# PereUbu7/Variational-Self-Organizing-Maps

Hardware: NVIDIA B200
Metric: train_samples_per_s (higher is better)
Workload: dtype f32

## Files before the change

### include/vsom_b200.h

```cpp
#ifndef VSOM_B200_H
#define VSOM_B200_H

#include <stddef.h>
#include <stdint.h>

#ifdef __cplusplus
extern "C" {
#endif

#if defined(__GNUC__)
#define VSOM_API __attribute__((visibility("default")))
#else
#define VSOM_API
#endif

typedef struct vsom_ctx vsom_ctx;

typedef enum vsom_status
{
    VSOM_OK = 0,
    VSOM_ERR_INVALID = -1,
    VSOM_ERR_CUDA = -2,
    VSOM_ERR_UNSUPPORTED = -3,
    VSOM_ERR_TIMEOUT = -4,
// ... 29 lines not shown
VSOM_API int vsom_peer_export_planes(vsom_ctx *ctx, unsigned char handle[64]);
VSOM_API int vsom_peer_import_planes(vsom_ctx *ctx, int rank, const unsigned char handle[64]);
VSOM_API int vsom_peer_attach(vsom_ctx *ctx, int rank, vsom_ctx *peer);
VSOM_API int vsom_shard_rows(const vsom_ctx *ctx, int *block_rows, int *local_rows, int *global_rows);
VSOM_API const char *vsom_last_error(const vsom_ctx *ctx);
VSOM_API int vsom_model_length(int d_in, int transform);
VSOM_API int vsom_depth(const vsom_ctx *ctx);
VSOM_API int vsom_node_count(const vsom_ctx *ctx);
VSOM_API void *vsom_stream(const vsom_ctx *ctx);
VSOM_API int vsom_synchronize(vsom_ctx *ctx);
VSOM_API uint64_t vsom_launch_count(const vsom_ctx *ctx);
VSOM_API int vsom_planes_resident(const vsom_ctx *ctx);

VSOM_API int vsom_debug_profile(vsom_ctx *ctx, int enable);
VSOM_API int vsom_debug_last_train_fast(const vsom_ctx *ctx);
VSOM_API int vsom_debug_phase_cycles(vsom_ctx *ctx, double out[5]);
VSOM_API int vsom_debug_phase_cycles_raw(vsom_ctx *ctx, double out[8]);
VSOM_API int vsom_debug_die_aware(const vsom_ctx *ctx);

VSOM_API int vsom_debug_measure_peaks(vsom_ctx *ctx, double out[4]);

VSOM_API int vsom_upload_state(vsom_ctx *ctx, const float *mean, const float *S, const float *sigma, const float *weight, const uint64_t *hits);
VSOM_API int vsom_download_state(vsom_ctx *ctx, float *mean, float *S, float *sigma, float *weight, uint64_t *hits);

#define VSOM_LINEAR_INIT_SLAB_ROWS 16384
VSOM_API int vsom_linear_init(vsom_ctx *ctx, const float *x, size_t n, double *out_mean, double *out_lambda, double *out_axes);
VSOM_API int vsom_debug_linear_init_phases(const vsom_ctx *ctx, double out[4]);

#define VSOM_CLUSTER_BLOCK 1024
typedef enum vsom_cluster_weighting
// ... 52 lines not shown
```

### variational-self-organizing-maps_b200/binding.py

```python
from __future__ import annotations

import ctypes as C
import os
import re

import numpy as np

from . import build as _build

STANDARD, MEDIAN, CLR = 0, 1, 2
EXPONENTIAL, INVERSE_PROPORTIONAL = 0, 1
ORDER_REFERENCE, ORDER_LANES, ORDER_EIGEN_SSE = 0, 1, 2
CLUSTER_UNIFORM, CLUSTER_HITS = 0, 1

_f32p = C.POINTER(C.c_float)
_f64p = C.POINTER(C.c_double)
_u32p = C.POINTER(C.c_uint32)
_u64p = C.POINTER(C.c_uint64)
_i32p = C.POINTER(C.c_int32)
_vp = C.c_void_p

_PROTOS = {
    "vsom_create": (C.c_int, [C.POINTER(_vp), C.c_int, C.c_int, C.c_int, C.c_int, C.c_int, C.c_int]),
    "vsom_destroy": (None, [_vp]),
# ... 2 lines not shown
    "vsom_peer_import": (C.c_int, [_vp, C.c_int, C.c_char_p]),
    "vsom_peer_export_planes": (C.c_int, [_vp, C.c_char_p]),
    "vsom_peer_import_planes": (C.c_int, [_vp, C.c_int, C.c_char_p]),
    "vsom_peer_attach": (C.c_int, [_vp, C.c_int, _vp]),
    "vsom_shard_rows": (C.c_int, [_vp, C.POINTER(C.c_int), C.POINTER(C.c_int), C.POINTER(C.c_int)]),
    "vsom_last_error": (C.c_char_p, [_vp]),
    "vsom_model_length": (C.c_int, [C.c_int, C.c_int]),
    "vsom_depth": (C.c_int, [_vp]),
    "vsom_node_count": (C.c_int, [_vp]),
    "vsom_stream": (_vp, [_vp]),
    "vsom_synchronize": (C.c_int, [_vp]),
    "vsom_launch_count": (C.c_uint64, [_vp]),
    "vsom_planes_resident": (C.c_int, [_vp]),
    "vsom_debug_profile": (C.c_int, [_vp, C.c_int]),
    "vsom_debug_last_train_fast": (C.c_int, [_vp]),
    "vsom_debug_phase_cycles_raw": (C.c_int, [_vp, _f64p]),
    "vsom_debug_die_aware": (C.c_int, [_vp]),
    "vsom_debug_measure_peaks": (C.c_int, [_vp, _f64p]),
    "vsom_debug_phase_cycles": (C.c_int, [_vp, _f64p]),
    "vsom_upload_state": (C.c_int, [_vp, _f32p, _f32p, _f32p, _f32p, _u64p]),
    "vsom_download_state": (C.c_int, [_vp, _f32p, _f32p, _f32p, _f32p, _u64p]),
    "vsom_get_node": (C.c_int, [_vp, C.c_size_t, _f32p, _f32p]),
    "vsom_linear_init": (C.c_int, [_vp, _f32p, C.c_size_t, _f64p, _f64p, _f64p]),
    "vsom_debug_linear_init_phases": (C.c_int, [_vp, _f64p]),
    "vsom_debug_cluster_phases": (C.c_int, [_vp, _f64p]),
    "vsom_cluster_nodes": (C.c_int, [_vp, C.c_int, C.c_uint64, C.c_int, C.c_int, _i32p, _f64p, _f64p, _f64p, C.POINTER(C.c_int), C.POINTER(C.c_int)]),
    "vsom_train_chunk": (C.c_int, [_vp, _f32p, C.c_size_t, C.c_double, C.c_double, C.c_int, _u64p, _u32p, _f32p, _f32p]),
    "vsom_train_chunk_device": (C.c_int, [_vp, _vp, C.c_size_t, C.c_double, C.c_double, C.c_int, _vp, _vp]),
    "vsom_batch_epoch": (C.c_int, [_vp, _f32p, C.c_size_t, C.c_double, C.c_int, _u64p, _f32p]),
    "vsom_find_bmu": (C.c_int, [_vp, _f32p, C.c_size_t, C.c_uint64, _u32p, _f32p]),
# ... 350 lines not shown
        return dict(zip(names, out.tolist()))

    def measure_peaks(self):
        out = np.zeros(4, np.float64)
        self._check(lib().vsom_debug_measure_peaks(self._h, _p(out, _f64p)))
        return {"smem_gbs": out[0], "smem_gbs_per_sm": out[1], "l2_gbs": out[2], "l2_set_mib": out[3]}

    @property
    def die_aware(self) -> bool:
        return bool(lib().vsom_debug_die_aware(self._h))

    @property
    def last_train_fast(self) -> bool:
        return bool(lib().vsom_debug_last_train_fast(self._h))

    def synchronize(self):
        self._check(lib().vsom_synchronize(self._h))

    @property
    def stream(self) -> int:
        return int(lib().vsom_stream(self._h) or 0)

    @property
    def launch_count(self) -> int:
        return int(lib().vsom_launch_count(self._h))

    @property
    def planes_resident(self) -> bool:
        return bool(lib().vsom_planes_resident(self._h))
```

### variational-self-organizing-maps_b200/csrc/capi.cu

```cuda
#include "common.cuh"

#include <cstdlib>

#include <algorithm>
#include <cstdio>
#include <cstring>

namespace vsom
{

static std::string g_createError;

int set_error(vsom_ctx *ctx, int code, const std::string &msg)
{
    if (ctx)
        ctx->err = msg;
    else
        g_createError = msg;
    return code;
}

int cuda_fail(vsom_ctx *ctx, cudaError_t e, const char *what, const char *file, int line)
{
    char buf[512];
// ... 320 lines not shown
        }
    }
    if (ctx->stream)
        cudaStreamDestroy(ctx->stream);
    delete ctx;
}

const char *vsom_last_error(const vsom_ctx *ctx) { return ctx ? ctx->err.c_str() : g_createError.c_str(); }
int vsom_depth(const vsom_ctx *ctx) { return ctx ? ctx->Dm : 0; }
int vsom_node_count(const vsom_ctx *ctx) { return ctx ? ctx->N : 0; }
void *vsom_stream(const vsom_ctx *ctx) { return ctx ? static_cast<void *>(ctx->stream) : nullptr; }
uint64_t vsom_launch_count(const vsom_ctx *ctx) { return ctx ? ctx->launches : 0; }
int vsom_planes_resident(const vsom_ctx *ctx) { return ctx ? ctx->k1.resident : 0; }

int vsom_debug_last_train_fast(const vsom_ctx *ctx) { return ctx && ctx->lastPlan == &ctx->k1f ? 1 : 0; }

int vsom_debug_profile(vsom_ctx *ctx, int enable)
{
    if (!ctx)
        return VSOM_ERR_INVALID;
    VSOM_CUDA(ctx, cudaSetDevice(ctx->device));
    VSOM_CUDA(ctx, cudaStreamSynchronize(ctx->stream));
    if (enable && !ctx->profDev)
    {
        VSOM_CUDA(ctx, cudaMalloc(&ctx->profDev, sizeof(long long) * 8 * ctx->numSMs));
        VSOM_CUDA(ctx, cudaMemset(ctx->profDev, 0, sizeof(long long) * 8 * ctx->numSMs));
    }
    else if (!enable && ctx->profDev)
    {
        VSOM_CUDA(ctx, cudaFree(ctx->profDev));
// ... 618 lines not shown
```

### variational-self-organizing-maps_b200/csrc/common.cuh

```cuda
#pragma once

#include <cuda.h>
#include <cuda_runtime.h>
#include <stdint.h>

#include <cmath>
#include <string>
#include <vector>

#include "vsom_b200.h"

namespace vsom
{

typedef unsigned long long u64;

constexpr size_t kMaxGridY = 65535;

struct LutEntry
{
    double nw;
    float cexp;
    float nwf;
};
// ... 55 lines not shown
    const void *scanMap;
};

struct StepPlan
{
    void (*kernel[2])(const StepParams) = {};
    int grid = 0;
    int threads = 0;
    size_t smem = 0;
    size_t smemCap = 0;
    int resident = 0;
    int smStride = 0;
    int lanesPerNode = 0;
    int profStride = 0;
    unsigned char profFold[5] = {};
};

}

struct vsom_ctx
{
    int device = 0;
    int W = 0, H = 0, N = 0, Din = 0, Dm = 0, Dr = 0, P = 0;
    int rank = 0, world = 1;
    int localN = 0;
    int shardBlock = 0, localRows = 0;
    std::vector<int> localRowY;
    float *peerMean[8] = {};
    bool peerMeanOpened[8] = {};
    vsom::u64 *rankSlots = nullptr;
// ... 19 lines not shown
    int *errFlag = nullptr;
    vsom::LutEntry *lut = nullptr;
    size_t lutCap = 0;
    std::vector<vsom::LutEntry> lutHost;
    double lutEta = -1, lutSigma = -1;
    int lutW = 0, lutH = 0;
    void *stage[10] = {};
    size_t stageCap[10] = {};
    bool trainEnqueued = false;
    bool poisoned = false;
    unsigned long long tcStats[3] = {0, 0, 0};
    int lastScoreTier = 0;
    uint64_t launches = 0;
    vsom::StepPlan k1, k1f;
    const vsom::StepPlan *lastPlan = nullptr;
    unsigned *winTab = nullptr;
    double winSigma = -1;
    vsom::u64 *rowPool = nullptr;
    int *rowMeta = nullptr;
    int dieAware = 0;
    vsom::u64 *distTag = nullptr;
    int scanBufs = 0, scanSeg = 0, scanNSeg = 0;
    void *scanMapDev = nullptr;
    void *umTab = nullptr;
    int umTiles = 0;
    long long *profDev = nullptr;
    size_t profSamples = 0;
    double linInitPhase[4] = {};
    double clusterPhase[5] = {};
    std::string err;
// ... 565 lines not shown
```

### variational-self-organizing-maps_b200/csrc/online_step.cu

```cuda
#include "common.cuh"

#include <cmath>
#include <cstdlib>
#include <string>

namespace vsom
{

constexpr int kThreads = 1024;
constexpr int kWarps = kThreads / 32;
constexpr int kMaxSlotsPerLane = 5;
constexpr size_t kStaticSmem = 1024;

template <int TR>
__device__ __forceinline__ void update_element(float xv, float c, float nwf, float &m, float &S)
{
    auto stepper = [](float d) { return TR == VSOM_MEDIAN ? median_sign(d) : d; };
    const float d0 = stepper(__fsub_rn(xv, m));
    const float m1 = __fadd_rn(m, __fmul_rn(c, d0));
    const float d1 = stepper(__fsub_rn(xv, m1));
    S = __fadd_rn(S, __fmul_rn(nwf, __fmul_rn(d0, d1)));
    m = m1;
}

// ... 974 lines not shown
        return set_error(ctx, VSOM_ERR_INVALID, "online step: decay must be Exponential or InverseProportional");
    if (n == 0)
        return VSOM_OK;
    if (ctx->world > 1)
        for (int r = 0; r < ctx->world; ++r)
            if (!ctx->peerSlots[r])
                return set_error(ctx, VSOM_ERR_INVALID, "online step: sharded context without vsom_peer_import for every rank");
    if (ctx->poisoned)
        return set_error(ctx, VSOM_ERR_TIMEOUT, "online step: an earlier chunk of this context aborted (a CTA or a rank never published its key); "
                                                "the map and the cross-rank step counter are no longer consistent — re-create the context");
    int rc = build_lut(ctx, eta, sigma);
    if (rc)
        return rc;
    const bool fast = ctx->k1f.grid && n < (1ull << 32) - 1;
    const StepPlan &plan = fast ? ctx->k1f : ctx->k1;
    VSOM_CUDA(ctx, cudaMemsetAsync(ctx->errFlag, 0, sizeof(int), ctx->stream));

    StepParams p{};
    p.W = ctx->W;
    p.H = ctx->H;
    p.shardBlock = ctx->shardBlock;
    p.nodeCount = ctx->localN;
    p.order = ctx->order;
    p.world = ctx->world;
    p.rank = ctx->rank;
    p.rankSlots = ctx->rankSlots;
    for (int r = 0; r < 8; ++r)
        p.peerSlots[r] = ctx->peerSlots[r];
    p.stepBase = ctx->stepBase;
    p.Din = ctx->Din;
// ... 20 lines not shown
    p.timeoutCycles = 4000000000ll;
    {
        const char *e = getenv("VSOM_PEER_TIMEOUT_S");
        const double secs = e && atof(e) > 0 ? atof(e) : 60.0;
        p.peerTimeoutCycles = static_cast<long long>(secs * 2.0e9);
    }
    p.localSearch = localSearch ? 1 : 0;
    p.lastIn = lastInDev;
    p.prof = ctx->profDev;
    p.xVec = (ctx->Din % 4 == 0 && (reinterpret_cast<uintptr_t>(xDev) & 15) == 0) ? 1 : 0;
    p.resident = plan.resident;
    p.smStride = plan.smStride;
    p.lanesPerNode = plan.lanesPerNode;
    p.lutCount = ctx->lutW * ctx->lutH;
    const size_t lutBytes = sizeof(LutEntry) * static_cast<size_t>(p.lutCount);
    p.lutSmem = plan.smem + lutBytes <= plan.smemCap ? 1 : 0;
    rc = fast ? prepare_online_step_fast(ctx, p, sigma) : prepare_online_step(ctx, p);
    if (rc)
        return rc;

    void *args[] = {&p};
    VSOM_CUDA(ctx, cudaLaunchCooperativeKernel(reinterpret_cast<void *>(plan.kernel[p.prof ? 1 : 0]), dim3(plan.grid), dim3(plan.threads), args,
                                               plan.smem + (p.lutSmem ? lutBytes : 0), ctx->stream));
    ctx->lastPlan = &plan;
    ctx->profSamples = n;
    ctx->launches += 1;
    ctx->stepBase += n;
    return VSOM_OK;
}

}
```

### variational-self-organizing-maps_b200/csrc/online_step_fast.cu

```cuda
#include "common.cuh"

#include <algorithm>
#include <cmath>
#include <cstdio>
#include <cstdlib>
#include <mutex>

namespace vsom
{

constexpr int kFThreads = 512;
constexpr int kFWarps = kFThreads / 32;
constexpr int kFMaxSlotsPerLane = 5;
constexpr int kFMaxCtas = 32 * kFMaxSlotsPerLane;
constexpr size_t kFStaticSmem = 4096;
constexpr int kFPoolBlocks = 1024;
constexpr int kWalkReplicas = 1;

__device__ __forceinline__ void named_bar_sync(int id, int threads) { asm volatile("bar.sync %0, %1;" ::"r"(id), "r"(threads) : "memory"); }
__device__ __forceinline__ void cp_async_commit() { asm volatile("cp.async.commit_group;" ::: "memory"); }

__device__ __forceinline__ u64 pk(float2 v) { return (static_cast<u64>(__float_as_uint(v.y)) << 32) | __float_as_uint(v.x); }
__device__ __forceinline__ float2 unpk(u64 v) { return make_float2(__uint_as_float(static_cast<unsigned>(v)), __uint_as_float(static_cast<unsigned>(v >> 32))); }
__device__ __forceinline__ float2 sub2(float2 a, float2 b)
// ... 126 lines not shown
    float rest[8] = {0.f, 0.f, 0.f, 0.f, 0.f, 0.f, 0.f, 0.f};
    if (nrest)
    {
        const float4 u = r4[2 * n8], v = r4[2 * n8 + 1];
        rest[0] = u.x;
        rest[1] = u.y;
        rest[2] = u.z;
        rest[3] = u.w;
        rest[4] = v.x;
        rest[5] = v.y;
        rest[6] = v.z;
        rest[7] = v.w;
    }
    return acc.finish(rest, nrest);
}
__device__ __forceinline__ float chain_lanes8(const float *row, int Dr, int c)
{
    const int n8 = Dr >> 3;
    float a = 0.0f;
    const float *q = row + c;
    int b = 0;
    if (n8 >= 8)
    {
        float v[8], w[8];
#pragma unroll
        for (int j = 0; j < 8; ++j)
            v[j] = q[8 * j];
#pragma unroll 1
        for (b = 8; b + 8 <= n8; b += 8)
        {
// ... 2 lines not shown
                w[j] = q[8 * (b + j)];
#pragma unroll
            for (int j = 0; j < 8; ++j)
                a = __fadd_rn(a, v[j]);
#pragma unroll
            for (int j = 0; j < 8; ++j)
                v[j] = w[j];
        }
#pragma unroll
        for (int j = 0; j < 8; ++j)
            a = __fadd_rn(a, v[j]);
    }
#pragma unroll 1
    for (; b < n8; ++b)
        a = __fadd_rn(a, q[8 * b]);
    float r = __fadd_rn(a, __shfl_xor_sync(0xffffffffu, a, 4));
    const int nrest = Dr & 7;
    const float *rest = row + (n8 << 3);
    int k = 0;
    if (nrest >= 4)
    {
        r = __fadd_rn(r, rest[c & 3]);
        k = 4;
    }
    r = __fadd_rn(r, __shfl_xor_sync(0xffffffffu, r, 2));
    r = __fadd_rn(r, __shfl_xor_sync(0xffffffffu, r, 1));
    for (; k < nrest; ++k)
        r = __fadd_rn(r, rest[k]);
    return r;
}
__device__ __forceinline__ float chain_any(const float *row, int n16, int Dr, int eigen) { return eigen ? chain_terms_eigen(row, Dr) : chain_terms(row, n16); }

__device__ __forceinline__ float4 clr_terms4(const float4 a, const float4 b, const float4 xi, const float4 xj)
{
    float4 t;
    float r = clr_residual(a.x, b.x, xi.x, xj.x);
    t.x = __fmul_rn(r, r);
    r = clr_residual(a.y, b.y, xi.y, xj.y);
    t.y = __fmul_rn(r, r);
    r = clr_residual(a.z, b.z, xi.z, xj.z);
    t.z = __fmul_rn(r, r);
    r = clr_residual(a.w, b.w, xi.w, xj.w);
    t.w = __fmul_rn(r, r);
    return t;
}

__device__ __forceinline__ u64 make_key_xy(float d, unsigned x, unsigned y, unsigned tag)
{
    unsigned bits = __float_as_uint(d);
    if (d != d)
        bits = (x | y) == 0 ? 0u : 0x7fffffffu;
    return (static_cast<u64>(bits) << 32) | (static_cast<u64>(y) << 20) | (static_cast<u64>(x) << 8) | tag;
}

__device__ __forceinline__ unsigned ld_relaxed_gpu_u32(const unsigned *p)
{
    unsigned v;
    asm volatile("ld.relaxed.gpu.global.u32 %0, [%1];" : "=r"(v) : "l"(p) : "memory");
    return v;
}

template <int TR, int IPW, bool PROF>
__global__ void __launch_bounds__(kFThreads, 1) online_step_fast_kernel(const StepParams p)
{
    constexpr int NI = IPW > 0 ? IPW : 1;
    extern __shared__ __align__(16) unsigned char smemRaw[];
    __shared__ u64 *sRowPtr[2][kFMaxCtas];
    __shared__ u64 sWarpKey[kFWarps];
    __shared__ int sPend[2];
    __shared__ unsigned sBmu;
    __shared__ int sAbort;
    __shared__ long long sProf[8];

    const int G = gridDim.x, b = blockIdx.x, tid = threadIdx.x, lane = tid & 31, warp = tid >> 5;
// ... 28 lines not shown
    ushort4 *pairS = reinterpret_cast<ushort4 *>(sBase + (IPW > 0 ? 0 : static_cast<size_t>(Lmax) * rstride));
    float *gS = reinterpret_cast<float *>(pairS + (kClr ? 2 * (Ppad >> 2) : 0));
    LutEntry *lutS = reinterpret_cast<LutEntry *>(gS + (kClr ? 6 * Ppad : 0));
    if (kClr)
    {
        unsigned short *pt = reinterpret_cast<unsigned short *>(pairS);
        const unsigned short zeroAt = static_cast<unsigned short>(XS - 4);
        for (int q = tid; q < Ppad; q += kFThreads)
        {
            pt[q] = q < p.P ? p.pairI[q] : zeroAt;
            pt[Ppad + q] = q < p.P ? p.pairJ[q] : zeroAt;
        }
    }

    if (tid == 0)
    {
        unsigned smid;
        asm volatile("mov.u32 %0, %%smid;" : "=r"(smid));
        const int die = p.dieOfSm[smid & 255];
        const unsigned idx = atomicAdd(p.rowCtr + die, 1u);
        p.rowOf[b] = die * kFMaxCtas + static_cast<int>(idx);
        __threadfence();
        atomicAdd(p.rowCtr + 2, 1u);
        const long long b0 = clock64();
        while (ld_relaxed_gpu_u32(p.rowCtr + 2) < static_cast<unsigned>(G))
            if (clock64() - b0 > p.timeoutCycles)
            {
                *p.err = 1;
                break;
            }
        __threadfence();
    }
    if (p.lutSmem)
        for (int i = tid; i < p.lutCount; i += kFThreads)
            lutS[i] = p.lut[i];
    for (int i = tid; i < p.W; i += kFThreads)
        winX[i] = p.winTab[i];
    for (int i = tid; i < p.H; i += kFThreads)
        winY[i] = p.winTab[p.W + i];
    for (int l = tid; l < Lpad; l += kFThreads)
    {
        hitsS[l] = 0;
        touchedS[l] = 0;
    }
    for (int k = tid; k < 4 * XS; k += kFThreads)
        xs[k] = 0.0f;
    for (int k = tid; k < stride; k += kFThreads)
// ... 60 lines not shown
    const int myL = LPN == 8 ? tid >> 3 : tid, mySub = LPN == 8 ? tid & 7 : 0;
    const bool inScan = myL < L;
    const bool hasNode = inScan && mySub == 0;
    unsigned myX = 0, myY = 0;
    float myW = 0.0f;
    unsigned myTouched = 0;
    if (hasNode)
    {
        const unsigned node = static_cast<unsigned>(p.node0 + myL * G + b);
        myX = node % static_cast<unsigned>(p.W);
        myY = node / static_cast<unsigned>(p.W);
        myW = p.weight[static_cast<size_t>(myL) * G + b];
    }
    const float *myTerms = tBase + (inScan ? myL : 0) * stride;
    __syncthreads();
    for (int i = tid; i < 2 * G; i += kFThreads)
    {
        const int d = i >> 1, buf = i & 1;
        const int r = p.rowOf[d];
        sRowPtr[buf][d] = p.rowPool + static_cast<size_t>(p.rowBlocks[2 * r + buf]) * 256;
    }

    constexpr int kPrefetchWarp = kFWarps - 2;
    const float *xsrc = p.x;
    int xdst = 0;
    auto prefetch = [&]() {
        float *dst = xs + xdst;
        if (p.xVec)
        {
#pragma unroll 1
            for (int k = lane * 4; k < p.Din; k += 128)
                cp_async16(dst + k, xsrc + k);
        }
        else
        {
#pragma unroll 1
// ... 118 lines not shown
            key = warp_min_key(key);
            if (nSW > 1)
            {
                if (lane == 0)
                    sWarpKey[warp] = key;
                named_bar_sync(1, nSW * 32);
            }
            unsigned bxy = 0;
            bool abort = false;
            if (warp == 0)
            {
                if (nSW > 1)
                    key = warp_min_key(lane < nSW ? sWarpKey[lane] : ~0ull);
                if (PROF && tid == 0)
                    c2 = clock64();
                u64 *const *rp = sRowPtr[par];
#pragma unroll
                for (int j = 0; j < kFMaxSlotsPerLane; ++j)
                    if (lane + 32 * j < G)
                        st_relaxed_gpu(rp[lane + 32 * j] + b, key);
                const u64 *row = rp[b];
                const u64 filler = (~0ull << 8) | tag;
                u64 m;
                long long t0 = 0;
                if (p.pollDelay > 0)
                {
                    const long long w0 = clock64();
                    while (clock64() - w0 < p.pollDelay)
                        ;
                }
                for (unsigned round = 0;; ++round)
                {
                    u64 v[kFMaxSlotsPerLane];
#pragma unroll
                    for (int j = 0; j < kFMaxSlotsPerLane; ++j)
                    {
                        const int i = lane + 32 * j;
                        v[j] = i < G ? ld_relaxed_gpu(row + i) : filler;
                    }
                    m = ~0ull;
                    int ok = 1;
#pragma unroll
                    for (int j = 0; j < kFMaxSlotsPerLane; ++j)
                    {
                        ok &= (static_cast<unsigned>(v[j] & 0xff) == tag);
                        m = u64_min(m, v[j]);
                    }
                    if (__all_sync(0xffffffffu, ok))
                        break;
                    if ((round & 63) == 63)
                    {
                        if (t0 == 0)
                            t0 = clock64();
                        else if (__any_sync(0xffffffffu, clock64() - t0 > p.timeoutCycles))
                        {
                            abort = true;
                            break;
                        }
                    }
                }
                m = warp_min_key(m);
                bxy = static_cast<unsigned>(m >> 8) & 0xffffffu;
                if (p.localSearch && !abort)
                {
                    if (lane == 0)
                    {
                        const u64 *dt = p.distTag + (static_cast<size_t>(par) * kWalkReplicas + (b % kWalkReplicas)) * p.nodeCount;
                        const unsigned want = t + 1u;
                        const unsigned bmu = local_bmu_walk(
                            [&](u64 i) {
                                u64 w = ld_relaxed_gpu(dt + i);
                                if (static_cast<unsigned>(w) != want)
                                {
                                    const long long w0 = clock64();
                                    do
                                        w = ld_relaxed_gpu(dt + i);
// ... 235 lines not shown
            for (int k = lane; k < p.Dm; k += 32)
            {
                const int ks = kClr ? (k < p.P ? k : Ppad + (k - p.P)) : k;
                const float sv = sBase[l * rstride + ks];
                p.mean[g + k] = mBase[l * rstride + ks];
                p.S[g + k] = sv;
                if (vis)
                    p.sigma[g + k] = lazy_sigma(sv, w);
            }
        }
    if (PROF && p.prof && tid == 0)
        for (int i = 0; i < 8; ++i)
            p.prof[static_cast<size_t>(b) * 8 + i] = sProf[i];
}

__global__ void die_pingpong_kernel(u64 *f1, u64 *f2, int ctaA, int ctaB, int iters, u64 base, long long *out, int *smids)
{
    if (threadIdx.x != 0)
        return;
    const int b = blockIdx.x;
    if (b != ctaA && b != ctaB)
        return;
    unsigned smid;
    asm volatile("mov.u32 %0, %%smid;" : "=r"(smid));
    smids[b == ctaA ? 0 : 1] = static_cast<int>(smid);
    const long long t0 = clock64();
    const long long limit = 400000000ll;
    for (int t = 1; t <= iters; ++t)
    {
        const u64 v = base + t;
// ... 93 lines not shown
    return bytes;
}

typedef void (*FastKernel)(const StepParams);
static FastKernel pick_fast(int transform, int ipw, bool prof)
{
    if (transform == VSOM_CLR)
        return prof ? online_step_fast_kernel<VSOM_CLR, 0, true> : online_step_fast_kernel<VSOM_CLR, 0, false>;
#define VSOM_FK(TR, I) {online_step_fast_kernel<TR, I, false>, online_step_fast_kernel<TR, I, true>}
#define VSOM_FKS(TR) {VSOM_FK(TR, 0), VSOM_FK(TR, 1), VSOM_FK(TR, 2), VSOM_FK(TR, 4)}
    static const FastKernel table[2][4][2] = {VSOM_FKS(VSOM_STANDARD), VSOM_FKS(VSOM_MEDIAN)};
#undef VSOM_FKS
#undef VSOM_FK
    const int slot = ipw == 4 ? 3 : ipw;
    return table[transform == VSOM_MEDIAN ? 1 : 0][slot][prof ? 1 : 0];
}

struct DieMap
{
    bool tried = false, valid = false;
    int dieOfSm[256] = {};
    int count[2] = {0, 0};
};
static DieMap g_dieMap[64];
static std::mutex g_dieMapMutex;

static bool split_bimodal(std::vector<float> v, float &thr)
{
    if (v.size() < 8)
        return false;
// ... 233 lines not shown
    {
        FastKernel k = pick_fast(ctx->transform, ipw, prof != 0);
        if (cudaFuncSetAttribute(k, cudaFuncAttributeMaxDynamicSharedMemorySize, ctx->smemOptin - static_cast<int>(kFStaticSmem)) != cudaSuccess)
        {
            cudaGetLastError();
            return;
        }
        int perSm = 0;
        if (cudaOccupancyMaxActiveBlocksPerMultiprocessor(&perSm, k, kFThreads, bytes) != cudaSuccess || perSm < 1)
        {
            cudaGetLastError();
            return;
        }
        pl.kernel[prof] = k;
    }
    pl.grid = G;
    pl.threads = kFThreads;
    pl.smem = bytes;
    pl.smemCap = static_cast<size_t>(ctx->smemOptin) - kFStaticSmem;
    pl.resident = 1;
    pl.smStride = stride;
    pl.lanesPerNode = ctx->order == VSOM_ORDER_EIGEN_SSE && Lmax * 8 <= kFThreads && (Lmax * 8 <= 32 || ctx->Dr >= 256) ? 8 : 1;
    pl.profStride = 8;
    const unsigned char fold[5] = {0, 0x03, 0x04, 0x18, 0x60};
    std::copy(fold, fold + 5, pl.profFold);
    ctx->k1f = pl;
}

static int build_window_table(vsom_ctx *ctx, double sigma)
{
// ... 50 lines not shown
```

Baseline: 473,100.

## Add warp-specialized pipelined online step kernel with register-resident nodes

Adds a new cooperative online-training kernel that keeps each node's mean and S in registers, with two nodes per node warp. A dedicated exchange warp performs the cross-CTA BMU min-exchange while node warps prefetch samples through a cp.async ring and compute the next sample's distances, synchronising over named barriers. This is meant to overlap distance computation, sample loading and the global exchange latency, and to avoid shared-memory round trips for node state. It is only used for standard/median transforms with Eigen-SSE ordering, Dr a multiple of 8 up to 256, and small per-CTA node counts. It adds a large, complex code path with a separate reduction order that must match the existing one.

```diff
diff --git a/include/vsom_b200.h b/include/vsom_b200.h
--- a/include/vsom_b200.h
+++ b/include/vsom_b200.h
@@ -67,6 +67,7 @@
 
 VSOM_API int vsom_debug_profile(vsom_ctx *ctx, int enable);
 VSOM_API int vsom_debug_last_train_fast(const vsom_ctx *ctx);
+VSOM_API int vsom_debug_last_online_body(const vsom_ctx *ctx);
 VSOM_API int vsom_debug_phase_cycles(vsom_ctx *ctx, double out[5]);
 VSOM_API int vsom_debug_phase_cycles_raw(vsom_ctx *ctx, double out[8]);
 VSOM_API int vsom_debug_die_aware(const vsom_ctx *ctx);
diff --git a/variational-self-organizing-maps_b200/binding.py b/variational-self-organizing-maps_b200/binding.py
--- a/variational-self-organizing-maps_b200/binding.py
+++ b/variational-self-organizing-maps_b200/binding.py
@@ -40,6 +40,7 @@
     "vsom_planes_resident": (C.c_int, [_vp]),
     "vsom_debug_profile": (C.c_int, [_vp, C.c_int]),
     "vsom_debug_last_train_fast": (C.c_int, [_vp]),
+    "vsom_debug_last_online_body": (C.c_int, [_vp]),
     "vsom_debug_phase_cycles_raw": (C.c_int, [_vp, _f64p]),
     "vsom_debug_die_aware": (C.c_int, [_vp]),
     "vsom_debug_measure_peaks": (C.c_int, [_vp, _f64p]),
@@ -420,6 +421,10 @@
     def last_train_fast(self) -> bool:
         return bool(lib().vsom_debug_last_train_fast(self._h))
 
+    @property
+    def last_online_body(self):
+        return {0: "generic", 1: "fast", 2: "pipelined"}.get(int(lib().vsom_debug_last_online_body(self._h)))
+
     def synchronize(self):
         self._check(lib().vsom_synchronize(self._h))
 
diff --git a/variational-self-organizing-maps_b200/csrc/capi.cu b/variational-self-organizing-maps_b200/csrc/capi.cu
--- a/variational-self-organizing-maps_b200/csrc/capi.cu
+++ b/variational-self-organizing-maps_b200/csrc/capi.cu
@@ -358,6 +358,12 @@
 int vsom_planes_resident(const vsom_ctx *ctx) { return ctx ? ctx->k1.resident : 0; }
 
 int vsom_debug_last_train_fast(const vsom_ctx *ctx) { return ctx && ctx->lastPlan == &ctx->k1f ? 1 : 0; }
+int vsom_debug_last_online_body(const vsom_ctx *ctx)
+{
+    if (!ctx || !ctx->lastPlan)
+        return -1;
+    return ctx->lastPlan != &ctx->k1f ? 0 : ctx->lastPipelined ? 2 : 1;
+}
 
 int vsom_debug_profile(vsom_ctx *ctx, int enable)
 {
diff --git a/variational-self-organizing-maps_b200/csrc/common.cuh b/variational-self-organizing-maps_b200/csrc/common.cuh
--- a/variational-self-organizing-maps_b200/csrc/common.cuh
+++ b/variational-self-organizing-maps_b200/csrc/common.cuh
@@ -93,6 +93,8 @@
     int lanesPerNode = 0;
     int profStride = 0;
     unsigned char profFold[5] = {};
+    void (*pipelined[2])(const StepParams) = {};
+    size_t pipelinedSmem = 0;
 };
 
 }
@@ -142,6 +144,7 @@
     uint64_t launches = 0;
     vsom::StepPlan k1, k1f;
     const vsom::StepPlan *lastPlan = nullptr;
+    int lastPipelined = 0;
     unsigned *winTab = nullptr;
     double winSigma = -1;
     vsom::u64 *rowPool = nullptr;
diff --git a/variational-self-organizing-maps_b200/csrc/online_step.cu b/variational-self-organizing-maps_b200/csrc/online_step.cu
--- a/variational-self-organizing-maps_b200/csrc/online_step.cu
+++ b/variational-self-organizing-maps_b200/csrc/online_step.cu
@@ -1012,6 +1012,8 @@
         return rc;
     const bool fast = ctx->k1f.grid && n < (1ull << 32) - 1;
     const StepPlan &plan = fast ? ctx->k1f : ctx->k1;
+    const bool pipelined = fast && !localSearch && plan.pipelined[0];
+    const size_t smem = pipelined ? plan.pipelinedSmem : plan.smem;
     VSOM_CUDA(ctx, cudaMemsetAsync(ctx->errFlag, 0, sizeof(int), ctx->stream));
 
     StepParams p{};
@@ -1062,15 +1064,16 @@
     p.lanesPerNode = plan.lanesPerNode;
     p.lutCount = ctx->lutW * ctx->lutH;
     const size_t lutBytes = sizeof(LutEntry) * static_cast<size_t>(p.lutCount);
-    p.lutSmem = plan.smem + lutBytes <= plan.smemCap ? 1 : 0;
+    p.lutSmem = smem + lutBytes <= plan.smemCap ? 1 : 0;
     rc = fast ? prepare_online_step_fast(ctx, p, sigma) : prepare_online_step(ctx, p);
     if (rc)
         return rc;
 
     void *args[] = {&p};
-    VSOM_CUDA(ctx, cudaLaunchCooperativeKernel(reinterpret_cast<void *>(plan.kernel[p.prof ? 1 : 0]), dim3(plan.grid), dim3(plan.threads), args,
-                                               plan.smem + (p.lutSmem ? lutBytes : 0), ctx->stream));
+    VSOM_CUDA(ctx, cudaLaunchCooperativeKernel(reinterpret_cast<void *>((pipelined ? plan.pipelined : plan.kernel)[p.prof ? 1 : 0]), dim3(plan.grid),
+                                               dim3(plan.threads), args, smem + (p.lutSmem ? lutBytes : 0), ctx->stream));
     ctx->lastPlan = &plan;
+    ctx->lastPipelined = pipelined ? 1 : 0;
     ctx->profSamples = n;
     ctx->launches += 1;
     ctx->stepBase += n;
diff --git a/variational-self-organizing-maps_b200/csrc/online_step_fast.cu b/variational-self-organizing-maps_b200/csrc/online_step_fast.cu
--- a/variational-self-organizing-maps_b200/csrc/online_step_fast.cu
+++ b/variational-self-organizing-maps_b200/csrc/online_step_fast.cu
@@ -164,6 +164,22 @@
     }
     return acc.finish(rest, nrest);
 }
+__device__ __forceinline__ float eigen_lanes8_finish(float a, const float *rest, int nrest, int c)
+{
+    float r = __fadd_rn(a, __shfl_xor_sync(0xffffffffu, a, 4));
+    int k = 0;
+    if (nrest >= 4)
+    {
+        r = __fadd_rn(r, rest[c & 3]);
+        k = 4;
+    }
+    r = __fadd_rn(r, __shfl_xor_sync(0xffffffffu, r, 2));
+    r = __fadd_rn(r, __shfl_xor_sync(0xffffffffu, r, 1));
+    for (; k < nrest; ++k)
+        r = __fadd_rn(r, rest[k]);
+    return r;
+}
+
 __device__ __forceinline__ float chain_lanes8(const float *row, int Dr, int c)
 {
     const int n8 = Dr >> 3;
@@ -196,20 +212,7 @@
 #pragma unroll 1
     for (; b < n8; ++b)
         a = __fadd_rn(a, q[8 * b]);
-    float r = __fadd_rn(a, __shfl_xor_sync(0xffffffffu, a, 4));
-    const int nrest = Dr & 7;
-    const float *rest = row + (n8 << 3);
-    int k = 0;
-    if (nrest >= 4)
-    {
-        r = __fadd_rn(r, rest[c & 3]);
-        k = 4;
-    }
-    r = __fadd_rn(r, __shfl_xor_sync(0xffffffffu, r, 2));
-    r = __fadd_rn(r, __shfl_xor_sync(0xffffffffu, r, 1));
-    for (; k < nrest; ++k)
-        r = __fadd_rn(r, rest[k]);
-    return r;
+    return eigen_lanes8_finish(a, row + (n8 << 3), Dr & 7, c);
 }
 __device__ __forceinline__ float chain_any(const float *row, int n16, int Dr, int eigen) { return eigen ? chain_terms_eigen(row, Dr) : chain_terms(row, n16); }
 
@@ -240,6 +243,84 @@
     unsigned v;
     asm volatile("ld.relaxed.gpu.global.u32 %0, [%1];" : "=r"(v) : "l"(p) : "memory");
     return v;
+}
+
+__device__ __forceinline__ void claim_exchange_rows(const StepParams &p, int b, int G)
+{
+    unsigned smid;
+    asm volatile("mov.u32 %0, %%smid;" : "=r"(smid));
+    const int die = p.dieOfSm[smid & 255];
+    const unsigned idx = atomicAdd(p.rowCtr + die, 1u);
+    p.rowOf[b] = die * kFMaxCtas + static_cast<int>(idx);
+    __threadfence();
+    atomicAdd(p.rowCtr + 2, 1u);
+    const long long b0 = clock64();
+    while (ld_relaxed_gpu_u32(p.rowCtr + 2) < static_cast<unsigned>(G))
+        if (clock64() - b0 > p.timeoutCycles)
+        {
+            *p.err = 1;
+            break;
+        }
+    __threadfence();
+}
+
+__device__ __forceinline__ void load_exchange_rows(u64 *(&sRowPtr)[2][kFMaxCtas], const StepParams &p, int G, int tid)
+{
+    for (int i = tid; i < 2 * G; i += kFThreads)
+    {
+        const int d = i >> 1, buf = i & 1;
+        const int r = p.rowOf[d];
+        sRowPtr[buf][d] = p.rowPool + static_cast<size_t>(p.rowBlocks[2 * r + buf]) * 256;
+    }
+}
+
+__device__ __forceinline__ u64 exchange_min_key(u64 *const *rp, int b, int G, int lane, u64 key, unsigned tag, const StepParams &p, bool &abort)
+{
+#pragma unroll
+    for (int j = 0; j < kFMaxSlotsPerLane; ++j)
+        if (lane + 32 * j < G)
+            st_relaxed_gpu(rp[lane + 32 * j] + b, key);
+    const u64 *row = rp[b];
+    const u64 filler = (~0ull << 8) | tag;
+    u64 m;
+    long long t0 = 0;
+    if (p.pollDelay > 0)
+    {
+        const long long w0 = clock64();
+        while (clock64() - w0 < p.pollDelay)
+            ;
+    }
+    for (unsigned round = 0;; ++round)
+    {
+        u64 v[kFMaxSlotsPerLane];
+#pragma unroll
+        for (int j = 0; j < kFMaxSlotsPerLane; ++j)
+        {
+            const int i = lane + 32 * j;
+            v[j] = i < G ? ld_relaxed_gpu(row + i) : filler;
+        }
+        m = ~0ull;
+        int ok = 1;
+#pragma unroll
+        for (int j = 0; j < kFMaxSlotsPerLane; ++j)
+        {
+            ok &= (static_cast<unsigned>(v[j] & 0xff) == tag);
+            m = u64_min(m, v[j]);
+        }
+        if (__all_sync(0xffffffffu, ok))
+            break;
+        if ((round & 63) == 63)
+        {
+            if (t0 == 0)
+                t0 = clock64();
+            else if (__any_sync(0xffffffffu, clock64() - t0 > p.timeoutCycles))
+            {
+                abort = true;
+                break;
+            }
+        }
+    }
+    return warp_min_key(m);
 }
 
 template <int TR, int IPW, bool PROF>
@@ -298,23 +379,7 @@
     }
 
     if (tid == 0)
-    {
-        unsigned smid;
-        asm volatile("mov.u32 %0, %%smid;" : "=r"(smid));
-        const int die = p.dieOfSm[smid & 255];
-        const unsigned idx = atomicAdd(p.rowCtr + die, 1u);
-        p.rowOf[b] = die * kFMaxCtas + static_cast<int>(idx);
-        __threadfence();
-        atomicAdd(p.rowCtr + 2, 1u);
-        const long long b0 = clock64();
-        while (ld_relaxed_gpu_u32(p.rowCtr + 2) < static_cast<unsigned>(G))
-            if (clock64() - b0 > p.timeoutCycles)
-            {
-                *p.err = 1;
-                break;
-            }
-        __threadfence();
-    }
+        claim_exchange_rows(p, b, G);
     if (p.lutSmem)
         for (int i = tid; i < p.lutCount; i += kFThreads)
             lutS[i] = p.lut[i];
@@ -405,12 +470,7 @@
     }
     const float *myTerms = tBase + (inScan ? myL : 0) * stride;
     __syncthreads();
-    for (int i = tid; i < 2 * G; i += kFThreads)
-    {
-        const int d = i >> 1, buf = i & 1;
-        const int r = p.rowOf[d];
-        sRowPtr[buf][d] = p.rowPool + static_cast<size_t>(p.rowBlocks[2 * r + buf]) * 256;
-    }
+    load_exchange_rows(sRowPtr, p, G, tid);
 
     constexpr int kPrefetchWarp = kFWarps - 2;
     const float *xsrc = p.x;
@@ -559,52 +619,7 @@
                     key = warp_min_key(lane < nSW ? sWarpKey[lane] : ~0ull);
                 if (PROF && tid == 0)
                     c2 = clock64();
-                u64 *const *rp = sRowPtr[par];
-#pragma unroll
-                for (int j = 0; j < kFMaxSlotsPerLane; ++j)
-                    if (lane + 32 * j < G)
-                        st_relaxed_gpu(rp[lane + 32 * j] + b, key);
-                const u64 *row = rp[b];
-                const u64 filler = (~0ull << 8) | tag;
-                u64 m;
-                long long t0 = 0;
-                if (p.pollDelay > 0)
-                {
-                    const long long w0 = clock64();
-                    while (clock64() - w0 < p.pollDelay)
-                        ;
-                }
-                for (unsigned round = 0;; ++round)
-                {
-                    u64 v[kFMaxSlotsPerLane];
-#pragma unroll
-                    for (int j = 0; j < kFMaxSlotsPerLane; ++j)
-                    {
-                        const int i = lane + 32 * j;
-                        v[j] = i < G ? ld_relaxed_gpu(row + i) : filler;
-                    }
-                    m = ~0ull;
-                    int ok = 1;
-#pragma unroll
-                    for (int j = 0; j < kFMaxSlotsPerLane; ++j)
-                    {
-                        ok &= (static_cast<unsigned>(v[j] & 0xff) == tag);
-                        m = u64_min(m, v[j]);
-                    }
-                    if (__all_sync(0xffffffffu, ok))
-                        break;
-                    if ((round & 63) == 63)
-                    {
-                        if (t0 == 0)
-                            t0 = clock64();
-                        else if (__any_sync(0xffffffffu, clock64() - t0 > p.timeoutCycles))
-                        {
-                            abort = true;
-                            break;
-                        }
-                    }
-                }
-                m = warp_min_key(m);
+                const u64 m = exchange_min_key(sRowPtr[par], b, G, lane, key, tag, p, abort);
                 bxy = static_cast<unsigned>(m >> 8) & 0xffffffu;
                 if (p.localSearch && !abort)
                 {
@@ -870,6 +885,372 @@
             p.prof[static_cast<size_t>(b) * 8 + i] = sProf[i];
 }
 
+constexpr int kPNodeWarps = 14;
+constexpr int kPExchangeWarp = kFWarps - 1;
+constexpr int kPRing = 4;
+constexpr int kPBarBmu = 1, kPBarKeys = 2;
+constexpr unsigned kPAbortBit = 1u << 31;
+
+__device__ __forceinline__ void named_bar_arrive(int id, int threads) { asm volatile("bar.arrive %0, %1;" ::"r"(id), "r"(threads) : "memory"); }
+template <int N>
+__device__ __forceinline__ void cp_async_wait_group() { asm volatile("cp.async.wait_group %0;" ::"n"(N) : "memory"); }
+
+template <int BPG, bool PAD>
+__device__ __forceinline__ void sq_terms(const float (&m)[BPG], const float (&x)[BPG], const bool (&val)[BPG], float (&t)[BPG])
+{
+#pragma unroll
+    for (int j = 0; j < BPG; j += 2)
+    {
+        const float2 r = sub2(make_float2(m[j], m[j + 1]), make_float2(x[j], x[j + 1]));
+        const float2 q = mul2(r, r);
+        t[j] = !PAD || val[j] ? q.x : 0.0f;
+        t[j + 1] = !PAD || val[j + 1] ? q.y : 0.0f;
+    }
+}
+
+template <int BPG, int NN>
+__device__ __forceinline__ void chain_groups(const float (&t)[NN][BPG], float (&d)[NN], int grp, int c)
+{
+    float a[NN];
+#pragma unroll
+    for (int i = 0; i < NN; ++i)
+        a[i] = 0.0f;
+#pragma unroll
+    for (int g = 0; g < 4; ++g)
+    {
+        if (g > 0)
+#pragma unroll
+            for (int i = 0; i < NN; ++i)
+            {
+                const float up = __shfl_up_sync(0xffffffffu, a[i], 8);
+                if (grp == g)
+                    a[i] = up;
+            }
+        if (grp == g)
+#pragma unroll
+            for (int j = 0; j < BPG; ++j)
+#pragma unroll
+                for (int i = 0; i < NN; ++i)
+                    a[i] = __fadd_rn(a[i], t[i][j]);
+    }
+#pragma unroll
+    for (int i = 0; i < NN; ++i)
+        d[i] = eigen_lanes8_finish(a[i], nullptr, 0, c);
+}
+
+__device__ __forceinline__ long long clock_after(unsigned dep)
+{
+    long long v;
+    asm volatile("mov.u64 %0, %%clock64;" : "=l"(v) : "r"(dep) : "memory");
+    return v;
+}
+
+template <int TR, int BPG, bool PAD, bool PROF>
+__global__ void __launch_bounds__(kFThreads, 1) online_step_pipelined_kernel(const StepParams p)
+{
+    extern __shared__ __align__(16) unsigned char smemRaw[];
+    __shared__ u64 *sRowPtr[2][kFMaxCtas];
+    __shared__ u64 sKey[kPNodeWarps];
+    __shared__ unsigned sBmu;
+    __shared__ long long sProf[8], sPubT, sPostT;
+
+    const int G = gridDim.x, b = blockIdx.x, tid = threadIdx.x, lane = tid & 31, warp = tid >> 5;
+    const int Lmax = (p.nodeCount + G - 1) / G;
+    const int L = (p.nodeCount - b + G - 1) / G;
+    const int Lpad = (Lmax + 3) & ~3;
+    const int nNW = (Lmax + 1) >> 1;
+    const int barThreads = (nNW + 1) * 32;
+    const int n8 = p.Dr >> 3;
+    const unsigned n = static_cast<unsigned>(p.n);
+    const int grp = lane >> 3, c = lane & 7;
+
+    float *ring = reinterpret_cast<float *>(smemRaw);
+    unsigned *winX = reinterpret_cast<unsigned *>(ring + nNW * kPRing * BPG * 32);
+    const int Wpad = (p.W + 3) & ~3, Hpad = (p.H + 3) & ~3;
+    unsigned *winY = winX + Wpad;
+    float2 *coef = reinterpret_cast<float2 *>(winY + Hpad);
+    float *wS = reinterpret_cast<float *>(coef + Lpad);
+    unsigned *touchedS = reinterpret_cast<unsigned *>(wS + Lpad);
+    LutEntry *lutS = reinterpret_cast<LutEntry *>(touchedS + Lpad);
+
+    if (tid == 0)
+        claim_exchange_rows(p, b, G);
+    if (p.lutSmem)
+        for (int i = tid; i < p.lutCount; i += kFThreads)
+            lutS[i] = p.lut[i];
+    for (int i = tid; i < p.W; i += kFThreads)
+        winX[i] = p.winTab[i];
+    for (int i = tid; i < p.H; i += kFThreads)
+        winY[i] = p.winTab[p.W + i];
+    if (tid == 0)
+        for (int i = 0; i < 8; ++i)
+            sProf[i] = 0;
+
+    const bool isExchange = warp == kPExchangeWarp;
+    const bool eAct = isExchange && lane < L;
+    unsigned eX = 0, eY = 0, eTouched = 0, eHits = 0;
+    float eW = 0.0f;
+    if (eAct)
+    {
+        const unsigned node = static_cast<unsigned>(p.node0) + static_cast<unsigned>(lane * G + b);
+        eX = node % static_cast<unsigned>(p.W);
+        eY = node / static_cast<unsigned>(p.W);
+        eW = p.weight[static_cast<size_t>(lane) * G + b];
+    }
+    const bool isNode = warp < nNW;
+    bool val[BPG];
+#pragma unroll
+    for (int j = 0; j < BPG; ++j)
+        val[j] = grp * BPG + j < n8;
+    int nl[2];
+    bool nAct[2];
+    unsigned nX[2], nY[2];
+    float m[2][BPG], s[2][BPG];
+#pragma unroll
+    for (int i = 0; i < 2; ++i)
+    {
+        nl[i] = warp + nNW * i;
+        nAct[i] = isNode && nl[i] < L;
+        nX[i] = nY[i] = 0;
+#pragma unroll
+        for (int j = 0; j < BPG; ++j)
+            m[i][j] = s[i][j] = 0.0f;
+        if (nAct[i])
+        {
+            const size_t q = static_cast<size_t>(nl[i]) * G + b;
+            const unsigned node = static_cast<unsigned>(p.node0) + static_cast<unsigned>(q);
+            nX[i] = node % static_cast<unsigned>(p.W);
+            nY[i] = node / static_cast<unsigned>(p.W);
+#pragma unroll
+            for (int j = 0; j < BPG; ++j)
+                if (val[j])
+                {
+                    const size_t g = q * p.rowStride + 8 * (grp * BPG + j) + c;
+                    m[i][j] = p.mean[g];
+                    s[i][j] = p.S[g];
+                }
+        }
+    }
+    float *myRing = ring + (isNode ? warp : 0) * kPRing * BPG * 32 + lane;
+    if (isNode)
+#pragma unroll
+        for (int j = 0; j < BPG; ++j)
+            if (!val[j])
+                for (int r = 0; r < kPRing; ++r)
+                    myRing[(r * BPG + j) * 32] = 0.0f;
+    __syncthreads();
+    load_exchange_rows(sRowPtr, p, G, tid);
+    __syncthreads();
+
+    if (isExchange)
+    {
+        int lutW = p.lutW, lutInSmem = p.lutSmem, expDecay = p.decay == VSOM_EXPONENTIAL ? 1 : 0;
+        asm volatile("" : "+r"(lutW), "+r"(lutInSmem), "+r"(expDecay));
+        for (unsigned t = 0; t < n; ++t)
+        {
+            const unsigned tag = (t >> 1) & 0xffu;
+            named_bar_sync(kPBarKeys, barThreads);
+            const u64 wkey = lane < nNW ? sKey[lane] : ~0ull;
+            long long te = 0, tm = 0, tx = 0;
+            if (PROF)
+                te = clock_after(static_cast<unsigned>(wkey));
+            const u64 key = warp_min_key(wkey);
+            if (PROF)
+                tm = clock_after(static_cast<unsigned>(key));
+            bool abort = false;
+            const u64 mk = exchange_min_key(sRowPtr[t & 1u], b, G, lane, key, tag, p, abort);
+            if (PROF)
+                tx = clock_after(static_cast<unsigned>(mk));
+            const unsigned bxy = static_cast<unsigned>(mk >> 8) & 0xffffffu;
+            if (eAct && !abort)
+            {
+                const unsigned bx = bxy & 0xfffu, by = bxy >> 12;
+                const unsigned wx = winX[bx], wy = winY[by];
+                float2 cf = make_float2(0.0f, -1.0f);
+                if (eX >= (wx & 0xffffu) && eX < (wx >> 16) && eY >= (wy & 0xffffu) && eY < (wy >> 16))
+                {
+                    const int dx = eX > bx ? eX - bx : bx - eX, dy = eY > by ? eY - by : by - eY;
+                    cf = step_coefficient(neighbourhood_entry(lutInSmem, lutS, p.lut, lutW, dx, dy), expDecay, eW);
+                    eTouched = 1;
+                    eHits += (dx | dy) == 0 ? 1u : 0u;
+                }
+                coef[lane] = cf;
+            }
+            if (lane == 0)
+            {
+                sBmu = bxy | (abort ? kPAbortBit : 0u);
+                if (abort)
+                    *p.err = 1;
+                if (PROF)
+                {
+                    const long long tp = clock_after(sBmu);
+                    sProf[6] += te - sPostT;
+                    sProf[1] += tm - te;
+                    sProf[2] += tx - tm;
+                    sProf[3] += tp - tx;
+                    sPubT = tp;
+                }
+            }
+            named_bar_arrive(kPBarBmu, barThreads);
+            if (abort)
+                break;
+        }
+        if (eAct)
+        {
+            const size_t q = static_cast<size_t>(lane) * G + b;
+            p.weight[q] = eW;
+            if (eHits)
+                p.hits[q] += eHits;
+            wS[lane] = eW;
+            touchedS[lane] = eTouched;
+        }
+    }
+    else if (isNode)
+    {
+        auto fetch = [&](unsigned sIdx) {
+            if (sIdx < n)
+            {
+                const float *src = p.x + static_cast<size_t>(sIdx) * p.Din + c;
+                float *dst = myRing + (sIdx & (kPRing - 1)) * BPG * 32;
+#pragma unroll
+                for (int j = 0; j < BPG; ++j)
+                    if (val[j])
+                        cp_async4(dst + j * 32, src + 8 * (grp * BPG + j));
+            }
+            cp_async_commit();
+        };
+        auto read = [&](unsigned sIdx, float(&x)[BPG]) {
+            cp_async_wait_group<2>();
+            const float *src = myRing + (sIdx & (kPRing - 1)) * BPG * 32;
+#pragma unroll
+            for (int j = 0; j < BPG; ++j)
+                x[j] = src[j * 32];
+        };
+        auto post_key = [&](const float (&x)[BPG], unsigned tag) {
+            float tt[2][BPG], d[2];
+            sq_terms<BPG, PAD>(m[0], x, val, tt[0]);
+            sq_terms<BPG, PAD>(m[1], x, val, tt[1]);
+            chain_groups<BPG, 2>(tt, d, grp, c);
+            u64 k = nAct[0] ? make_key_xy(d[0], nX[0], nY[0], tag) : ~0ull;
+            if (nAct[1])
+                k = u64_min(k, make_key_xy(d[1], nX[1], nY[1], tag));
+            if (lane == 24)
+                sKey[warp] = k;
+        };
+        float xc[BPG], xn[BPG];
+        fetch(0);
+        fetch(1);
+        fetch(2);
+        read(0, xc);
+        post_key(xc, 0);
+        if (PROF && tid == 0)
+            sPostT = clock_after(0u);
+        named_bar_arrive(kPBarKeys, barThreads);
+        for (unsigned t = 0; t < n; ++t)
+        {
+            fetch(t + 3);
+            read(t + 1, xn);
+            named_bar_sync(kPBarBmu, barThreads);
+            const unsigned bw = sBmu;
+            long long tw = 0, tu = 0;
+            if (PROF)
+                tw = clock_after(bw);
+            if (bw & kPAbortBit)
+                break;
+            float2 cf[2];
+            bool in[2];
+#pragma unroll
+            for (int i = 0; i < 2; ++i)
+            {
+                cf[i] = coef[nAct[i] ? nl[i] : 0];
+                in[i] = nAct[i] && cf[i].y >= 0.0f;
+            }
+            auto update = [&](int i, int j) {
+                float2 mm = make_float2(m[i][j], m[i][j + 1]), ss = make_float2(s[i][j], s[i][j + 1]);
+                fast_update_pair<TR>(make_float2(xc[j], xc[j + 1]), cf[i].x, cf[i].y, mm, ss);
+                m[i][j] = mm.x;
+                m[i][j + 1] = mm.y;
+                s[i][j] = ss.x;
+                s[i][j + 1] = ss.y;
+            };
+            if (in[0] && in[1])
+            {
+#pragma unroll
+                for (int j = 0; j < BPG; j += 2)
+                {
+                    update(0, j);
+                    update(1, j);
+                }
+            }
+            else
+#pragma unroll
+                for (int i = 0; i < 2; ++i)
+                    if (in[i])
+#pragma unroll
+                        for (int j = 0; j < BPG; j += 2)
+                            update(i, j);
+            if (PROF)
+                tu = clock_after(__float_as_uint(m[0][0]) ^ __float_as_uint(m[1][BPG - 1]));
+            if (t + 1 < n)
+            {
+                post_key(xn, ((t + 1) >> 1) & 0xffu);
+                if (PROF && tid == 0)
+                {
+                    const long long tk = clock_after(0u);
+                    sProf[4] += tw - sPubT;
+                    sProf[5] += tu - tw;
+                    sProf[0] += tk - tu;
+                    sPostT = tk;
+                }
+                named_bar_arrive(kPBarKeys, barThreads);
+            }
+            const unsigned bx = bw & 0xfffu, by = bw >> 12;
+#pragma unroll
+            for (int i = 0; i < 2; ++i)
+                if (in[i] && nX[i] == bx && nY[i] == by)
+                {
+                    float tt[1][BPG], d[1];
+                    sq_terms<BPG, PAD>(m[i], xc, val, tt[0]);
+                    chain_groups<BPG, 1>(tt, d, grp, c);
+                    if (lane == 24)
+                    {
+                        if (p.outBmu)
+                            p.outBmu[t] = static_cast<unsigned>(p.node0) + static_cast<unsigned>(nl[i] * G + b);
+                        if (p.outDist)
+                            p.outDist[t] = d[0];
+                    }
+                }
+#pragma unroll
+            for (int j = 0; j < BPG; ++j)
+                xc[j] = xn[j];
+        }
+        cp_async_wait_all();
+    }
+
+    __syncthreads();
+#pragma unroll
+    for (int i = 0; i < 2; ++i)
+        if (nAct[i])
+        {
+            const size_t q = static_cast<size_t>(nl[i]) * G + b;
+            const bool vis = touchedS[nl[i]] != 0;
+            const float w = wS[nl[i]];
+#pragma unroll
+            for (int j = 0; j < BPG; ++j)
+                if (val[j])
+                {
+                    const size_t g = q * p.rowStride + 8 * (grp * BPG + j) + c;
+                    p.mean[g] = m[i][j];
+                    p.S[g] = s[i][j];
+                    if (vis)
+                        p.sigma[g] = lazy_sigma(s[i][j], w);
+                }
+        }
+    if (PROF && p.prof && tid == 0)
+        for (int i = 0; i < 8; ++i)
+            p.prof[static_cast<size_t>(b) * 8 + i] = sProf[i];
+}
+
 __global__ void die_pingpong_kernel(u64 *f1, u64 *f2, int ctaA, int ctaB, int iters, u64 base, long long *out, int *smids)
 {
     if (threadIdx.x != 0)
@@ -993,6 +1374,35 @@
 #undef VSOM_FK
     const int slot = ipw == 4 ? 3 : ipw;
     return table[transform == VSOM_MEDIAN ? 1 : 0][slot][prof ? 1 : 0];
+}
+
+static FastKernel pick_pipelined(int transform, int bpg, bool pad, bool prof)
+{
+#define VSOM_PK(TR, B, P) {online_step_pipelined_kernel<TR, B, P, false>, online_step_pipelined_kernel<TR, B, P, true>}
+#define VSOM_PKS(TR) {{VSOM_PK(TR, 4, false), VSOM_PK(TR, 4, true)}, {VSOM_PK(TR, 8, false), VSOM_PK(TR, 8, true)}}
+    static const FastKernel table[2][2][2][2] = {VSOM_PKS(VSOM_STANDARD), VSOM_PKS(VSOM_MEDIAN)};
+#undef VSOM_PKS
+#undef VSOM_PK
+    return table[transform == VSOM_MEDIAN ? 1 : 0][bpg == 8 ? 1 : 0][pad ? 1 : 0][prof ? 1 : 0];
+}
+
+static int pipelined_bpg(const vsom_ctx *ctx, int G)
+{
+    if ((ctx->transform != VSOM_STANDARD && ctx->transform != VSOM_MEDIAN) || ctx->order != VSOM_ORDER_EIGEN_SSE)
+        return 0;
+    if (ctx->Dr % 8 != 0 || ctx->Dr > 256 || ctx->Dr != ctx->Din || fast_ipw(ctx, G) == 0)
+        return 0;
+    if ((ctx->localN + G - 1) / G > 2 * kPNodeWarps)
+        return 0;
+    return ctx->Dr <= 128 ? 4 : 8;
+}
+
+static size_t pipelined_smem(const vsom_ctx *ctx, int G, int bpg)
+{
+    const int Lmax = (ctx->localN + G - 1) / G;
+    const int nNW = (Lmax + 1) >> 1;
+    const size_t Wpad = (ctx->W + 3) & ~3, Hpad = (ctx->H + 3) & ~3, Lpad = (Lmax + 3) & ~3;
+    return sizeof(float) * static_cast<size_t>(nNW) * kPRing * bpg * 32 + sizeof(unsigned) * (Wpad + Hpad) + (sizeof(float2) + sizeof(float) + sizeof(unsigned)) * Lpad;
 }
 
 struct DieMap
@@ -1256,6 +1666,25 @@
         }
         pl.kernel[prof] = k;
     }
+    const int bpg = pipelined_bpg(ctx, G);
+    if (bpg)
+    {
+        const size_t pbytes = pipelined_smem(ctx, G, bpg);
+        for (int prof = 0; prof < 2; ++prof)
+        {
+            FastKernel k = pick_pipelined(ctx->transform, bpg, ctx->Dr != 32 * bpg, prof != 0);
+            int perSm = 0;
+            if (cudaFuncSetAttribute(k, cudaFuncAttributeMaxDynamicSharedMemorySize, ctx->smemOptin - static_cast<int>(kFStaticSmem)) != cudaSuccess ||
+                cudaOccupancyMaxActiveBlocksPerMultiprocessor(&perSm, k, kFThreads, pbytes) != cudaSuccess || perSm < 1)
+            {
+                cudaGetLastError();
+                pl.pipelined[0] = pl.pipelined[1] = nullptr;
+                break;
+            }
+            pl.pipelined[prof] = k;
+        }
+        pl.pipelinedSmem = pbytes;
+    }
     pl.grid = G;
     pl.threads = kFThreads;
     pl.smem = bytes;
```

Result: faster. 613,600 (median of 6 runs) (+29.7%).
